# leaner-forever/SEGS-SLAM

Measured on AMD Instinct MI355X. Metric: mapper train-iters/sec (fwd+bwd raster), higher is better.
Workload: dtype f32; 1 GPU; 1080p_3m: 3000000 Gaussians, 1920x1080, 1 keyframe per GPU, fwd+bwd raster; P=3000000, P_visible=2096178, num_rendered=10472370, instances_binned=7913347, instances_live=6766534, width=1920, height=1080, parallelism=keyframe-dp1, forward=resident (no host sync), hipgraph=off

## Files before the change

### include/segs_raster.h

```cpp
#ifndef SEGS_RASTER_H_
#define SEGS_RASTER_H_

#include <stddef.h>
#include <stdint.h>

#ifdef __cplusplus
extern "C" {
#endif

#define SEGS_OK 0
#define SEGS_ERR_INVALID_ARGUMENT (-1)
#define SEGS_ERR_UNSUPPORTED (-2)
#define SEGS_ERR_ALLOC (-3)

typedef char* (*segs_alloc_fn)(void* ctx, size_t bytes);

const char* segs_last_error(void);

#define SEGS_RASTER_SKIP_NONPOSITIVE_OPACITY 1u
#define SEGS_RASTER_KEEP_DEAD_INSTANCES 2u
#define SEGS_RASTER_GATHER_TILES_TOUCHED 4u
#define SEGS_RASTER_TEST_NARROW_PACK 8u
#define SEGS_RASTER_UNFUSED_BINNING 16u
#define SEGS_RASTER_TIGHT_BINNING 32u
#define SEGS_RASTER_MFMA_MOMENTS 64u
#define SEGS_RASTER_NO_WRITTEN_BYTES 128u
uint32_t segs_raster_set_flags(uint32_t flags);

uint32_t* segs_raster_set_status_mirror(uint32_t* host_mapped_status);

size_t segs_geometry_bytes(int P);
size_t segs_image_bytes(int width, int height);
size_t segs_binning_bytes(int num_rendered);

int segs_rasterize_forward(segs_alloc_fn geometry_alloc, void* geometry_ctx,
                           segs_alloc_fn binning_alloc, void* binning_ctx,
                           segs_alloc_fn image_alloc, void* image_ctx,
                           int P, int D, int M,
                           const float* background, int width, int height,
                           const float* means3D, const float* shs, const float* colors_precomp,
                           const float* opacities, const float* scales, float scale_modifier,
                           const float* rotations, const float* cov3D_precomp,
                           const float* viewmatrix, const float* projmatrix, const float* cam_pos,
                           float tan_fovx, float tan_fovy, int prefiltered,
                           float* out_color, int* radii, void* stream, int* num_rendered);

int segs_rasterize_backward(int P, int D, int M, int R,
                            const float* background, int width, int height,
                            const float* means3D, const float* shs, const float* colors_precomp,
                            const float* scales, float scale_modifier, const float* rotations,
                            const float* cov3D_precomp, const float* viewmatrix, const float* projmatrix,
                            const float* campos, float tan_fovx, float tan_fovy, const int* radii,
                            char* geom_buffer, char* binning_buffer, char* image_buffer,
                            const float* dL_dpix, float* dL_dmean2D, float* dL_dconic, float* dL_dopacity,
                            float* dL_dcolor, float* dL_dmean3D, float* dL_dcov3D, float* dL_dsh,
                            float* dL_dscale, float* dL_drot, void* stream);

int segs_visible_filter(int P, int M, int width, int height, const float* means3D, const float* scales,
                        float scale_modifier, const float* rotations, const float* cov3D_precomp,
// ... 167 lines not shown
```

### segs-slam_amd/csrc/capi.hip

```cpp
#include <hip/hip_runtime.h>
#include <cstdio>
#include <cstdlib>
#include <algorithm>
#include <cstring>
#include <string>
#include <vector>
#include "../../include/segs_raster.h"
#include "gs_layout.h"
#include "kernels.h"
#include "capi_args.h"

using namespace segs;

namespace {
thread_local std::string g_err;
}
int segs::set_error(int code, const char* what) {
  g_err = what;
  return code;
}
int segs::set_hip_error(hipError_t e, const char* where) {
  g_err = std::string(where) + ": " + hipGetErrorString(e);
  return (int)e > 0 ? (int)e : 1;
}
// ... 261 lines not shown
      S.ranges(), S.point_list(), V.width, V.height, S.G.rec(), background, S.final_T(), S.n_contrib(), dL_dpix, S.G.gacc(), V.tiles, written);
  LAUNCH_TRY("render_bwd_kernel");
  return SEGS_OK;
}

int camera_grads_begin(const segs_camera_grads* cam, const float* shs, bool empty, hipStream_t st, bool* live) {
  *live = false;
  if (!cam) return SEGS_OK;
  if (!cam->dL_dviewmatrix || !cam->dL_dprojmatrix || !cam->temp) return fail(SEGS_ERR_INVALID_ARGUMENT, "segs_camera_grads: null field");
  if (shs) return fail(SEGS_ERR_INVALID_ARGUMENT, "camera gradients need colors_precomp: the SH colours depend on campos, which they do not cover");
  if (empty) {
    HIP_TRY(hipMemsetAsync(cam->dL_dviewmatrix, 0, 16 * sizeof(float), st));
    HIP_TRY(hipMemsetAsync(cam->dL_dprojmatrix, 0, 16 * sizeof(float), st));
    return SEGS_OK;
  }
  *live = true;
  return SEGS_OK;
}
float* camera_partials(const segs_camera_grads* cam) { return (float*)align_ptr(cam->temp); }
int camera_grads_finish(const segs_camera_grads* cam, int nblocks, hipStream_t st) {
  camera_grad_reduce_kernel<<<1, 960, 0, st>>>(camera_partials(cam), nblocks, cam->dL_dviewmatrix, cam->dL_dprojmatrix);
  LAUNCH_TRY("camera_grad_reduce_kernel");
  return SEGS_OK;
}

int launch_preprocess_bwd(const Gaussians& g, const View& V, const int* radii, const GradOutputs& o, const PerGaussianBwd& m, hipStream_t st) {
  const bool depth = m.depth || m.dz_in;
  auto* const kernel = m.cam ? (depth ? preprocess_bwd_kernel<true, true> : preprocess_bwd_kernel<false, true>)
                             : (depth ? preprocess_bwd_kernel<true, false> : preprocess_bwd_kernel<false, false>);
  const int nblocks = (g.P + 255) / 256;
  kernel<<<nblocks, 256, 0, st>>>(g.P, g.means3D, radii, g.kernel_scales(), g.rotations, g.scale_modifier, g.cov3D_precomp, V.viewmatrix,
                                  V.projmatrix, V.focal_x, V.focal_y, V.tan_fovx, V.tan_fovy, m.gacc, (float)V.width, (float)V.height,
                                  o.dL_dmean2D, o.dL_dconic, o.dL_dopacity, o.dL_dcolor, o.dL_dmean3D, o.dL_dcov3D, o.dL_dscale, o.dL_drot,
                                  m.clean_gacc ? 1 : 0, m.dz_in, m.cam ? camera_partials(m.cam) : nullptr, m.written);
  LAUNCH_TRY("preprocess_bwd_kernel");
  return m.cam ? camera_grads_finish(m.cam, nblocks, st) : SEGS_OK;
}

int rasterize_forward(const Allocators& A, const Gaussians& g, const View& V, const float* background, float* out_color, int* radii,
                      const segs_depth_outputs* dout, hipStream_t st, int* num_rendered) {
  const int P = g.P;
  if (!A.geometry_alloc || !A.binning_alloc || !A.image_alloc) return fail(SEGS_ERR_INVALID_ARGUMENT, "null allocator callback");
  if (P < 0 || V.width <= 0 || V.height <= 0) return fail(SEGS_ERR_INVALID_ARGUMENT, "bad P / image size");
  if (P > MAX_GAUSSIANS) return fail(SEGS_ERR_INVALID_ARGUMENT, "P exceeds 2^28 Gaussians (sort values carry a 4-bit quadrant mask)");
  if (!background || !out_color || !V.viewmatrix || !V.projmatrix || !num_rendered) return fail(SEGS_ERR_INVALID_ARGUMENT, "null required pointer");
  if (P > 0 && (!g.means3D || !g.opacities)) return fail(SEGS_ERR_INVALID_ARGUMENT, "null means3D/opacities");
  if (P > 0)
    if (int rc = check_colour_and_shape(g, V)) return rc;
  if (int rc = check_tile_grid(V)) return rc;

  Scratch S{};
  char* geom_raw = A.geometry_alloc(A.geometry_ctx, geom_layout(P).total);
  S.IL = image_layout(V.width, V.height);
  char* img_raw = A.image_alloc(A.image_ctx, S.IL.total);
  if (!geom_raw || !img_raw) return fail(SEGS_ERR_ALLOC, "allocator callback returned null");
  S.G = geom_at(geom_raw, P);
  S.img = align_ptr(img_raw);
  const Geom& G = S.G;
  if (!radii) radii = G.radii_internal();

  int R = 0;
  uint32_t hdr[3] = {0u, 0u, 0u};
  const bool tight = (g_flags & SEGS_RASTER_TIGHT_BINNING) != 0u;
  bool fast_keys = tight;
  if (P > 0) {
    K1Targets k1;
    k1.extra_flags = tight ? PREPROCESS_TIGHT_RECT : 0u;
// ... 62 lines not shown
  }
  if (int rc = run_binning(S, V, BinningMode::resident_keys(keys.keys, drop_dead_instances()), st)) return rc;
  return launch_render_fwd(S, V, background, out_color, dout, st);
}

int rasterize_backward(const Gaussians& g, const View& V, const ScratchBuffers& B, const BackwardInputs& in, const GradOutputs& o,
                       GaccCleaning cleaning, hipStream_t st) {
  const int P = g.P, R = B.capacity;
  const bool self_clean = cleaning == SELF_CLEAN;
  if (P < 0 || R < 0 || V.width <= 0 || V.height <= 0) return fail(SEGS_ERR_INVALID_ARGUMENT, "bad sizes");
  if (B.geom_rows < P) return fail(SEGS_ERR_INVALID_ARGUMENT, "geom_rows must be >= P");
  bool cam_live = false;
  if (int rc = camera_grads_begin(in.cam, g.shs, P == 0 || R == 0, st, &cam_live)) return rc;
  if (P == 0) return SEGS_OK;
  if (g.shs && (!V.cam_pos || !o.dL_dsh || g.M <= 0)) return fail(SEGS_ERR_INVALID_ARGUMENT, "SH path needs campos, dL_dsh and M > 0");
  if (!B.geom_buffer || !B.binning_buffer || !B.image_buffer || !in.dL_dpix || !in.background || !g.means3D || !V.viewmatrix || !V.projmatrix)
    return fail(SEGS_ERR_INVALID_ARGUMENT, "null required pointer");
  if (!o.dL_dmean2D || !o.dL_dopacity || !o.dL_dcolor || !o.dL_dmean3D || (g.cov3D_precomp && !o.dL_dcov3D))
    return fail(SEGS_ERR_INVALID_ARGUMENT, "null gradient output");
  if (!g.cov3D_precomp && (!g.scales || !g.rotations || !o.dL_dscale || !o.dL_drot))
    return fail(SEGS_ERR_INVALID_ARGUMENT, "need scales+rotations (+ their gradient outputs) or cov3D_precomp");
  uint32_t* const no_status = nullptr;
  const Scratch S = carve(B, P, V, no_status);
  const Geom& G = S.G;
  const int* radii = in.radii ? in.radii : G.radii_internal();

  if (!self_clean) { PROF(K_MEMSET);
  HIP_TRY(hipMemsetAsync(G.gacc(), 0, (size_t)P * GACC_DWORDS * 4, st));
  }
  PerGaussianBwd m;
  m.gacc = G.gacc(); m.depth = in.dgrad && in.dgrad->dL_ddepth; m.clean_gacc = self_clean;
  if (cam_live) m.cam = in.cam;
  m.written = (self_clean && !(g_flags & SEGS_RASTER_NO_WRITTEN_BYTES)) ? G.written() : nullptr;
  if (R > 0)
    if (int rc = launch_render_bwd(S, V, in.background, in.dL_dpix, in.dgrad, m.written, st)) return rc;
  { PROF(K_PREPROCESS_BWD);
  if (int rc = launch_preprocess_bwd(g, V, radii, o, m, st)) return rc;
  }
  if (g.shs) {
    sh_backward_kernel<<<G.L.nblocks, 256, 0, st>>>(P, g.means3D, radii, g.shs, g.D, g.M, V.cam_pos, G.clamped(), o.dL_dcolor, o.dL_dmean3D, o.dL_dsh);
    LAUNCH_TRY("sh_backward_kernel");
  }
  return SEGS_OK;
}

int visible_filter(const Gaussians& g, const View& V, int log_scale_stride, int* radii, hipStream_t st) {
  if (g.P < 0 || V.width <= 0 || V.height <= 0) return fail(SEGS_ERR_INVALID_ARGUMENT, "bad sizes");
  if (g.P == 0) return SEGS_OK;
  if (!g.means3D || !V.viewmatrix || !V.projmatrix || !radii) return fail(SEGS_ERR_INVALID_ARGUMENT, "null required pointer");
  if (!g.cov3D_precomp && (!g.scales || !g.rotations)) return fail(SEGS_ERR_INVALID_ARGUMENT, "need scales+rotations or cov3D_precomp");
  visible_filter_kernel<<<(g.P + 255) / 256, 256, 0, st>>>(g.P, g.means3D, g.kernel_scales(), g.scale_modifier, g.rotations, g.cov3D_precomp,
                                                           V.viewmatrix, V.projmatrix, V.width, V.height, V.tan_fovx, V.tan_fovy, V.focal_x,
                                                           V.focal_y, V.gx, V.gy, radii, log_scale_stride);
  LAUNCH_TRY("visible_filter_kernel");
  return SEGS_OK;
}

int debug_preprocess_backward(const Gaussians& g, const View& V, const int* radii, const GradOutputs& o, const float* dL_dz,
                              const segs_camera_grads* cam, hipStream_t st) {
  bool cam_live = false;
  if (int rc = camera_grads_begin(cam, g.shs, g.P <= 0, st, &cam_live)) return rc;
  if (g.P <= 0) return SEGS_OK;
  if (!g.means3D || !radii || !V.viewmatrix || !V.projmatrix || !o.dL_dmean2D || !o.dL_dconic || !o.dL_dmean3D || !o.dL_dcov3D)
    return fail(SEGS_ERR_INVALID_ARGUMENT, "null pointer");
  PerGaussianBwd m;
  if (cam_live) { m.dz_in = dL_dz; m.cam = cam; }
  return launch_preprocess_bwd(g, V, radii, o, m, st);
}

}

extern "C" {

const char* segs_last_error(void) { return g_err.c_str(); }

uint32_t* segs_raster_set_status_mirror(uint32_t* host_mapped_status) {
  uint32_t* old = g_status_mirror;
  g_status_mirror = host_mapped_status;
  return old;
}

uint32_t segs_raster_set_flags(uint32_t flags) {
  const uint32_t old = g_flags;
  g_flags = flags;
  return old;
}

size_t segs_geometry_bytes(int P) { return geom_layout(P < 0 ? 0 : P).total; }
size_t segs_image_bytes(int width, int height) { return image_layout(width, height).total; }

int segs_debug_geometry_layout(int P, size_t* offset_and_bytes, int regions) {
  if (P < 0 || !offset_and_bytes || regions != SEGS_GEOMETRY_REGIONS) return fail(SEGS_ERR_INVALID_ARGUMENT, "bad P / region count");
  const GeomLayout g = geom_layout(P);
  const size_t p = (size_t)P;
  const size_t v[SEGS_GEOMETRY_REGIONS][2] = {
      {g.rec, p * REC_DWORDS * 4}, {g.bin, p * sizeof(BinInfo)}, {g.offsets, p * 4}, {g.radii_internal, p * 4},
      {g.block_sums, (size_t)(g.nblocks + 1) * 4 * 3}, {g.clamped, p * 4}, {g.num_rendered, 64}, {g.gacc, p * GACC_DWORDS * 4},
      {g.touched, p * 4}, {g.written, p}};
  for (int i = 0; i < SEGS_GEOMETRY_REGIONS; i++) { offset_and_bytes[2 * i] = v[i][0]; offset_and_bytes[2 * i + 1] = v[i][1]; }
// ... 382 lines not shown
```

### segs-slam_amd/csrc/capi_args.h

```cpp
#pragma once
#include <hip/hip_runtime.h>
#include <cstdint>
#include "../../include/segs_raster.h"
#include "gs_layout.h"
#include "kernels.h"

namespace segs {

struct Gaussians {
  int P; const float *means3D, *scales; float scale_modifier; const float *rotations, *cov3D_precomp;
  int D, M; const float *shs, *colors_precomp, *opacities;
  const float* kernel_scales() const { return cov3D_precomp ? nullptr : scales; }
};

struct View {
  int width, height; const float *viewmatrix, *projmatrix, *cam_pos; float tan_fovx, tan_fovy;
  uint32_t gx, gy, tiles; float focal_x, focal_y;
};
inline View image_view(int width, int height) {
  View v{};
  v.width = width; v.height = height;
  v.gx = (width + TILE_X - 1) / TILE_X; v.gy = (height + TILE_Y - 1) / TILE_Y; v.tiles = v.gx * v.gy;
  return v;
}
// ... 74 lines not shown
struct BinningMode {
  uint32_t dmin; int dbits; uint32_t dcull;
  int digit_bits;
  const uint32_t* k1_keys;
  bool drop_dead;
  static constexpr int RESIDENT_DIGIT_BITS = 9;
  static BinningMode resident_keys(const uint32_t* k1_keys, bool drop_dead) {
    return BinningMode{DEPTH_KEY_MIN, DEPTH_KEY_BITS, 0xFFFFFFFFu, RESIDENT_DIGIT_BITS, k1_keys, drop_dead};
  }
  static BinningMode exact_range(uint32_t max_not_depth, uint32_t max_depth, bool drop_dead) {
    const uint32_t dmin = ~max_not_depth, dspan = max_depth - dmin + 1u;
    int dbits = 1;
    while (dbits < 32 && (dspan >> dbits) != 0u) dbits++;
    const bool nine = (dbits + 8) / 9 < (dbits + 7) / 8;
    return BinningMode{dmin, dbits, dmin + dspan, nine ? 9 : 8, nullptr, drop_dead};
  }
};
inline DepthSortInput resident_depth_sort_input(char* bin, const GaussSortLayout& GS) { return depth_sort_input(bin, GS, DEPTH_KEY_BITS, BinningMode::RESIDENT_DIGIT_BITS); }

struct K1Targets {
  uint32_t *depth_keys = nullptr, *depth_vals = nullptr;
  uint2* ranges = nullptr;
  uint32_t extra_flags = 0u;
  uint32_t* depth_overflow = nullptr;
};

struct PerGaussianBwd {
  float* gacc = nullptr;
  bool depth = false;
  bool clean_gacc = false;
  const float* dz_in = nullptr;
  const segs_camera_grads* cam = nullptr;
  uint8_t* written = nullptr;
};

struct Allocators { segs_alloc_fn geometry_alloc; void* geometry_ctx; segs_alloc_fn binning_alloc; void* binning_ctx; segs_alloc_fn image_alloc; void* image_ctx; };

enum GaccCleaning { MEMSET_PER_CALL, SELF_CLEAN };
struct BackwardInputs { const float* background; const int* radii; const float* dL_dpix; const segs_depth_grads* dgrad; const segs_camera_grads* cam; };

constexpr const Gaussians* K1_RAN_AT_PRODUCER = nullptr;
constexpr const segs_depth_outputs* NO_DEPTH_OUTPUTS = nullptr;
constexpr const segs_depth_grads* NO_DEPTH_GRADS = nullptr;
constexpr const segs_camera_grads* NO_CAMERA_GRADS = nullptr;
constexpr const float *NO_CAM_POS = nullptr, *NO_DL_DZ = nullptr;
constexpr int* NO_RADII = nullptr;

}
```

### segs-slam_amd/csrc/kernels.h

```cpp
#pragma once
#include <hip/hip_runtime.h>
#include <cstdint>
#include "gs_layout.h"

namespace segs {

int set_error(int code, const char* what);
int set_hip_error(hipError_t e, const char* where);


__global__ void preprocess_fwd_kernel(
    int P, const float* __restrict__ means3D, const float* __restrict__ scales, float mod,
    const float* __restrict__ rotations, const float* __restrict__ opacities, const float* __restrict__ colors,
    const float* __restrict__ cov3D_precomp, const float* __restrict__ viewmatrix, const float* __restrict__ projmatrix,
    int W, int H, float tan_fovx, float tan_fovy, float focal_x, float focal_y, uint32_t gx, uint32_t gy,
    int* __restrict__ radii, float* __restrict__ rec, BinInfo* __restrict__ bin, uint32_t* __restrict__ block_sums,
    uint32_t* __restrict__ depth_range, const float* __restrict__ shs, int D, int M, const float* __restrict__ cam_pos,
    uint32_t* __restrict__ clamped, uint32_t flags, uint32_t* __restrict__ depth_keys, uint32_t* __restrict__ depth_vals,
    uint2* __restrict__ ranges, int num_tiles, uint32_t* __restrict__ depth_overflow, uint32_t* __restrict__ touched_dense);
constexpr uint32_t DEPTH_KEY_MIN = 0x3E4CCCCDu;
constexpr int DEPTH_KEY_BITS = 27;

__global__ void visible_filter_kernel(
    int P, const float* __restrict__ means3D, const float* __restrict__ scales, float mod,
    const float* __restrict__ rotations, const float* __restrict__ cov3D_precomp,
    const float* __restrict__ viewmatrix, const float* __restrict__ projmatrix, int W, int H,
    float tan_fovx, float tan_fovy, float focal_x, float focal_y, uint32_t gx, uint32_t gy, int* __restrict__ radii,
    int log_scale_stride);

__global__ void mark_visible_kernel(int P, const float* __restrict__ means3D, const float* __restrict__ viewmatrix,
                                    uint8_t* __restrict__ present);

constexpr int CAM_SUMS = 24;
template <bool DEPTH, bool CAM>
__global__ void preprocess_bwd_kernel(
    int P, const float* __restrict__ means3D, const int* __restrict__ radii, const float* __restrict__ scales,
    const float* __restrict__ rotations, float mod, const float* __restrict__ cov3D_precomp,
    const float* __restrict__ view, const float* __restrict__ proj, float h_x, float h_y, float tan_fovx, float tan_fovy,
    float* __restrict__ gacc, float img_w, float img_h,
    float* __restrict__ dL_dmean2D, float* __restrict__ dL_dconic,
    float* __restrict__ dL_dopacity, float* __restrict__ dL_dcolor, float* __restrict__ dL_dmean3D,
    float* __restrict__ dL_dcov3D, float* __restrict__ dL_dscale, float* __restrict__ dL_drot, int clean_gacc,
    const float* __restrict__ dz_in, float* __restrict__ cam_partials, uint8_t* __restrict__ written);
__global__ void camera_grad_reduce_kernel(const float* __restrict__ partials, int nblocks, float* __restrict__ dL_dview,
                                          float* __restrict__ dL_dproj);
__global__ void sh_backward_kernel(int P, const float* __restrict__ means3D, const int* __restrict__ radii,
                                   const float* __restrict__ shs, int D, int M, const float* __restrict__ cam_pos,
                                   const uint32_t* __restrict__ clamped, const float* __restrict__ dL_dcolor,
                                   float* __restrict__ dL_dmean3D, float* __restrict__ dL_dsh);

__global__ void scan_block_sums_kernel(uint32_t* __restrict__ block_sums, int nblocks, const uint32_t* __restrict__ depth_range,
                                       uint32_t* __restrict__ total);
__global__ void ordered_offsets_kernel(int P, const uint32_t* __restrict__ block_sums, uint32_t* __restrict__ incl,
                                       uint32_t* __restrict__ total_out, const uint32_t* __restrict__ ng_dev,
                                       uint32_t* __restrict__ first_owner, uint32_t owner_entries);
__global__ void duplicate_with_keys_kernel(int P, int R, const float* __restrict__ rec,
                                           const uint32_t* __restrict__ order, const uint32_t* __restrict__ incl,
                                           uint32_t* __restrict__ keys, uint32_t* __restrict__ vals, uint32_t gx,
                                           const uint32_t* __restrict__ n_dev, int mark_dead, const uint32_t* __restrict__ ng_dev,
                                           const uint32_t* __restrict__ first_owner);
constexpr uint32_t RANGE_EMPTY_START = 0xFFFFFFFFu;
__global__ void normalize_ranges_kernel(int num_tiles, uint2* __restrict__ ranges);
constexpr uint32_t PREPROCESS_TIGHT_RECT = 0x80000000u;
constexpr uint32_t DEAD_KEY = 0xFFFFFFFFu;
template <typename K, int BITS>
__global__ void radix_count_kernel(const K* __restrict__ keys, int n, int shift, uint32_t dmin, int dbits,
                                   uint32_t* __restrict__ tile_prefix, uint32_t* __restrict__ chunk_hist, int nblocks, int nchunks,
                                   const uint32_t* __restrict__ n_dev, int drop_dead, int chunk_tiles, int nbits);
__global__ void radix_scan_kernel(uint32_t* __restrict__ block_hist, int nblocks, uint32_t* __restrict__ digit_totals);
template <typename K, int BITS, bool AUX>
__global__ void radix_scatter_kernel(const K* __restrict__ keys_in, const uint32_t* __restrict__ vals_in,
                                     K* __restrict__ keys_out, uint32_t* __restrict__ vals_out, int n, int shift,
                                     uint32_t dmin, int dbits, const uint32_t* __restrict__ tile_prefix, const uint32_t* __restrict__ chunk_prefix,
                                     const uint32_t* __restrict__ digit_totals, int nblocks, int nchunks,
                                     const uint32_t* __restrict__ n_dev, int drop_dead, uint32_t* __restrict__ n_live_out,
                                     const uint32_t* __restrict__ aux_in, uint32_t* __restrict__ aux_out, int nbits, int chunk_tiles, int pack_shift,
// ... 47 lines not shown
```

### segs-slam_amd/csrc/preprocess.hip

```cpp
#include <hip/hip_runtime.h>
#include <cstdint>
#include "gs_layout.h"
#include "kernels.h"
#include "project_gaussian.h"
#include "sh_color.h"

#pragma clang fp contract(off)

namespace segs {

__device__ __forceinline__ float3 load_row3(const float* __restrict__ a, int P, float* lds ) {
  const int tid = threadIdx.x;
  const size_t base = (size_t)blockIdx.x * 768;
  const size_t lim = (size_t)P * 3;
#pragma unroll
  for (int k = 0; k < 3; k++) {
    const size_t i = base + k * 256 + tid;
    lds[k * 256 + tid] = i < lim ? a[i] : 0.f;
  }
  __syncthreads();
  float3 v = make_float3(lds[3 * tid], lds[3 * tid + 1], lds[3 * tid + 2]);
  __syncthreads();
  return v;
}

__device__ __forceinline__ void load_rows3(const float* __restrict__ a0, const float* __restrict__ a1, const float* __restrict__ a2,
                                           int P, float* lds , float3& v0, float3& v1, float3& v2) {
  const int tid = threadIdx.x;
  const size_t base = (size_t)blockIdx.x * 768;
  const size_t lim = (size_t)P * 3;
  const float* arr[3] = {a0, a1, a2};
  float t[3][3];
#pragma unroll
  for (int m = 0; m < 3; m++)
#pragma unroll
    for (int k = 0; k < 3; k++) {
      const size_t i = base + k * 256 + tid;
      t[m][k] = (arr[m] && i < lim) ? arr[m][i] : 0.f;
    }
#pragma unroll
  for (int m = 0; m < 3; m++)
#pragma unroll
    for (int k = 0; k < 3; k++) lds[m * 768 + k * 256 + tid] = t[m][k];
  __syncthreads();
  v0 = make_float3(lds[3 * tid], lds[3 * tid + 1], lds[3 * tid + 2]);
  v1 = make_float3(lds[768 + 3 * tid], lds[768 + 3 * tid + 1], lds[768 + 3 * tid + 2]);
  v2 = make_float3(lds[1536 + 3 * tid], lds[1536 + 3 * tid + 1], lds[1536 + 3 * tid + 2]);
  __syncthreads();
}

__global__ void __launch_bounds__(256) preprocess_fwd_kernel(
    int P, const float* __restrict__ means3D, const float* __restrict__ scales, float mod,
    const float* __restrict__ rotations, const float* __restrict__ opacities, const float* __restrict__ colors,
    const float* __restrict__ cov3D_precomp, const float* __restrict__ viewmatrix, const float* __restrict__ projmatrix,
    int W, int H, float tan_fovx, float tan_fovy, float focal_x, float focal_y, uint32_t gx, uint32_t gy,
    int* __restrict__ radii, float* __restrict__ rec, BinInfo* __restrict__ bin, uint32_t* __restrict__ block_sums,
    uint32_t* __restrict__ depth_range ,
    const float* __restrict__ shs, int D, int M, const float* __restrict__ cam_pos, uint32_t* __restrict__ clamped,
    uint32_t flags, uint32_t* __restrict__ depth_keys, uint32_t* __restrict__ depth_vals, uint2* __restrict__ ranges,
    int num_tiles, uint32_t* __restrict__ depth_overflow ,
    uint32_t* __restrict__ touched_dense) {
  __shared__ float lds[3 * 768];
  __shared__ uint32_t wave_sums[4], wave_dmax[4], wave_dnmin[4];
  const int idx = blockIdx.x * 256 + threadIdx.x;
  float4 rot = make_float4(0, 0, 0, 0);
  if (scales && idx < P) rot = reinterpret_cast<const float4*>(rotations)[idx];
  float3 p, sc, col;
  load_rows3(means3D, scales, colors, P, lds, p, sc, col);

  uint32_t touched = 0, dbits_mine = 0;
  float4 rq0 = make_float4(0, 0, 0, 0), rq1 = rq0, rq2 = rq0, rq3 = rq0;
  bool has_record = false;
  if (idx < P) {
    Projected g = project_gaussian(p, sc, mod, rot, cov3D_precomp ? cov3D_precomp + (size_t)6 * idx : nullptr,
                                   viewmatrix, projmatrix, W, H, tan_fovx, tan_fovy, focal_x, focal_y, gx, gy);
    if ((flags & 1u) && !(opacities[idx] > 0.f)) g.radius = 0;
    BinInfo b{0u, 0u, 0u, 0u};
    if (g.radius > 0) {
      const float op = opacities[idx];
      if (!colors) {
        uint32_t cb;
        col = sh::to_rgb(idx, D, M, p, cam_pos, shs, &cb);
// ... 92 lines not shown
__global__ void __launch_bounds__(256) mark_visible_kernel(int P, const float* __restrict__ means3D,
                                                           const float* __restrict__ viewmatrix, uint8_t* __restrict__ present) {
  __shared__ float lds[768];
  const int idx = blockIdx.x * 256 + threadIdx.x;
  const float3 p = load_row3(means3D, P, lds);
  if (idx >= P) return;
  float3 p_view = transformPoint4x3(p, viewmatrix);
  present[idx] = (p_view.z <= 0.2f) ? 0 : 1;
}

__device__ __forceinline__ void store_row3(float* __restrict__ a, int P, float* lds , float x, float y, float z) {
  const int tid = threadIdx.x;
  lds[3 * tid] = x; lds[3 * tid + 1] = y; lds[3 * tid + 2] = z;
  __syncthreads();
  const size_t base = (size_t)blockIdx.x * 768;
  const size_t lim = (size_t)P * 3;
#pragma unroll
  for (int k = 0; k < 3; k++) {
    const size_t i = base + k * 256 + tid;
    if (i < lim) a[i] = lds[k * 256 + tid];
  }
  __syncthreads();
}

struct Sym2 { float xx, xy, yy; };

__device__ __forceinline__ void quat_rows(float4 q, float R[3][3]) {
  const float r = q.x, x = q.y, y = q.z, z = q.w;
  R[0][0] = 1.f - 2.f * (y * y + z * z); R[0][1] = 2.f * (x * y - r * z);       R[0][2] = 2.f * (x * z + r * y);
  R[1][0] = 2.f * (x * y + r * z);       R[1][1] = 1.f - 2.f * (x * x + z * z); R[1][2] = 2.f * (y * z - r * x);
  R[2][0] = 2.f * (x * z - r * y);       R[2][1] = 2.f * (y * z + r * x);       R[2][2] = 1.f - 2.f * (x * x + y * y);
}

template <bool DEPTH, bool CAM>
__global__ void __launch_bounds__(256) preprocess_bwd_kernel(
    int P, const float* __restrict__ means3D, const int* __restrict__ radii, const float* __restrict__ scales,
    const float* __restrict__ rotations, float mod, const float* __restrict__ cov3D_precomp,
    const float* __restrict__ view, const float* __restrict__ proj, float h_x, float h_y, float tan_fovx, float tan_fovy,
    float* __restrict__ gacc, float img_w, float img_h,
    float* __restrict__ dL_dmean2D, float* __restrict__ dL_dconic,
    float* __restrict__ dL_dopacity, float* __restrict__ dL_dcolor, float* __restrict__ dL_dmean3D,
    float* __restrict__ dL_dcov3D, float* __restrict__ dL_dscale, float* __restrict__ dL_drot,
    int clean_gacc ,
    const float* __restrict__ dz_in, float* __restrict__ cam_partials ,
    uint8_t* __restrict__ written) {
  __shared__ float lds[3 * 768];
  const int idx = blockIdx.x * 256 + threadIdx.x;
  const bool live = idx < P;
  const bool row_written = (gacc && written) ? (live && written[idx] != 0) : live;
  const bool binned = live && radii[idx] > 0 && row_written;
  float3 mean, scale, unused;
  load_rows3(means3D, scales, nullptr, P, lds, mean, scale, unused);

  float g2x = 0.f, g2y = 0.f;
  Sym2 G{0.f, 0.f, 0.f};
  float dcol0 = 0.f, dcol1 = 0.f, dcol2 = 0.f, dop = 0.f, dz = 0.f;
  float4 a0 = make_float4(0.f, 0.f, 0.f, 0.f), a1 = a0;
  if (gacc) {
    {
      __shared__ __attribute__((aligned(16))) float gl[4][32 * GACC_DWORDS];
      const int lane = threadIdx.x & 63;
      float* const wl = gl[threadIdx.x >> 6];
      const uint64_t rows = __ballot(written ? row_written : binned);
      const size_t wave_first = (size_t)blockIdx.x * 256 + (threadIdx.x & ~63);
      if (written && clean_gacc && rows != 0ull && lane < 16 && wave_first + 4 * lane < (size_t)P)
        reinterpret_cast<uint32_t*>(written + wave_first)[lane] = 0u;
#pragma unroll
      for (int half = 0; half < 2; half++) {
        float4 q[2];
#pragma unroll
        for (int j = 0; j < 2; j++) {
          const int r = 16 * j + (lane >> 2), owner = 32 * half + r;
          q[j] = make_float4(0.f, 0.f, 0.f, 0.f);
          if (((rows >> owner) & 1ull) && (lane & 3) < 3) {
            float4* src = reinterpret_cast<float4*>(gacc + (wave_first + owner) * GACC_DWORDS) + (lane & 3);
            q[j] = *src;
            if (clean_gacc) *src = make_float4(0.f, 0.f, 0.f, 0.f);
          }
        }
#pragma unroll
        for (int j = 0; j < 2; j++) reinterpret_cast<float4*>(wl + (16 * j + (lane >> 2)) * GACC_DWORDS)[lane & 3] = q[j];
        asm volatile("" ::: "memory");
        if ((lane >> 5) == half) {
          const float4* mine = reinterpret_cast<const float4*>(wl + (lane & 31) * GACC_DWORDS);
          a0 = mine[0]; a1 = mine[1]; dcol2 = wl[(lane & 31) * GACC_DWORDS + 8];
          if (DEPTH) dz = wl[(lane & 31) * GACC_DWORDS + 9];
        }
        asm volatile("" ::: "memory");
      }
    }
    if (binned) {
      G.xx = -0.5f * a0.z; G.xy = -0.5f * a0.w; G.yy = -0.5f * a1.x;
      dop = a1.y;
      dcol0 = a1.z; dcol1 = a1.w;
    }
    store_row3(dL_dcolor, P, lds, dcol0, dcol1, dcol2);
    if (live) {
      if (dL_dconic) reinterpret_cast<float4*>(dL_dconic)[idx] = make_float4(G.xx, G.xy, 0.f, G.yy);
      dL_dopacity[idx] = dop;
    }
  } else if (live) {
    g2x = dL_dmean2D[3 * (size_t)idx + 0]; g2y = dL_dmean2D[3 * (size_t)idx + 1];
    G.xx = dL_dconic[4 * (size_t)idx + 0]; G.xy = dL_dconic[4 * (size_t)idx + 1]; G.yy = dL_dconic[4 * (size_t)idx + 3];
    if constexpr (CAM && DEPTH) { if (dz_in) dz = dz_in[idx]; }
  }

  float out_mean[3] = {0, 0, 0}, out_cov[6] = {0, 0, 0, 0, 0, 0}, out_scale[3] = {0, 0, 0}, out_rot[4] = {0, 0, 0, 0};
  float cam[CAM ? CAM_SUMS : 1] = {0};
  if (binned) {
    const float tx0 = view[0] * mean.x + view[4] * mean.y + view[8] * mean.z + view[12];
    const float ty0 = view[1] * mean.x + view[5] * mean.y + view[9] * mean.z + view[13];
    const float tz = view[2] * mean.x + view[6] * mean.y + view[10] * mean.z + view[14];
    const float limx = 1.3f * tan_fovx, limy = 1.3f * tan_fovy;
    const float rx = tx0 / tz, ry = ty0 / tz;
    const bool free_x = !(rx < -limx || rx > limx), free_y = !(ry < -limy || ry > limy);
    const float tx = fminf(limx, fmaxf(-limx, rx)) * tz, ty = fminf(limy, fmaxf(-limy, ry)) * tz;
    const float iz = 1.f / tz, iz2 = iz * iz;
    const float J00 = h_x * iz, J02 = -h_x * tx * iz2, J11 = h_y * iz, J12 = -h_y * ty * iz2;
    float M2[2][3];
#pragma unroll
    for (int j = 0; j < 3; j++) {
      M2[0][j] = J00 * view[4 * j] + J02 * view[4 * j + 2];
      M2[1][j] = J11 * view[4 * j + 1] + J12 * view[4 * j + 2];
    }
    float R[3][3] = {{0, 0, 0}, {0, 0, 0}, {0, 0, 0}}, s3[3] = {0, 0, 0};
    float4 q = make_float4(0, 0, 0, 0);
    float E[2][3];
    float U[2][3] = {{0, 0, 0}, {0, 0, 0}};
    float a, b, c;
    if (cov3D_precomp) {
      const float* cv = cov3D_precomp + (size_t)6 * idx;
      const float S[3][3] = {{cv[0], cv[1], cv[2]}, {cv[1], cv[3], cv[4]}, {cv[2], cv[4], cv[5]}};
#pragma unroll
      for (int r = 0; r < 2; r++)
#pragma unroll
        for (int j = 0; j < 3; j++) E[r][j] = M2[r][0] * S[0][j] + M2[r][1] * S[1][j] + M2[r][2] * S[2][j];
      a = E[0][0] * M2[0][0] + E[0][1] * M2[0][1] + E[0][2] * M2[0][2] + 0.3f;
      b = E[0][0] * M2[1][0] + E[0][1] * M2[1][1] + E[0][2] * M2[1][2];
      c = E[1][0] * M2[1][0] + E[1][1] * M2[1][1] + E[1][2] * M2[1][2] + 0.3f;
    } else {
      q = reinterpret_cast<const float4*>(rotations)[idx];
      quat_rows(q, R);
      s3[0] = mod * scale.x; s3[1] = mod * scale.y; s3[2] = mod * scale.z;
#pragma unroll
      for (int r = 0; r < 2; r++)
#pragma unroll
        for (int k = 0; k < 3; k++) U[r][k] = (M2[r][0] * R[0][k] + M2[r][1] * R[1][k] + M2[r][2] * R[2][k]) * s3[k];
#pragma unroll
      for (int r = 0; r < 2; r++)
#pragma unroll
        for (int j = 0; j < 3; j++) E[r][j] = U[r][0] * R[j][0] * s3[0] + U[r][1] * R[j][1] * s3[1] + U[r][2] * R[j][2] * s3[2];
      a = U[0][0] * U[0][0] + U[0][1] * U[0][1] + U[0][2] * U[0][2] + 0.3f;
      b = U[0][0] * U[1][0] + U[0][1] * U[1][1] + U[0][2] * U[1][2];
      c = U[1][0] * U[1][0] + U[1][1] * U[1][1] + U[1][2] * U[1][2] + 0.3f;
    }
    const float det = a * c - b * b;
    const float k = 1.0f / (det * det + 0.0000001f);
    if (gacc) {
      const float di = 1.0f / det;
      const float cA = c * di, cB = -b * di, cC = a * di;
      g2x = -(cA * a0.x + cB * a0.y) * (0.5f * img_w);
      g2y = -(cC * a0.y + cB * a0.x) * (0.5f * img_h);
    }
    const float h0 = c * G.xx - b * G.xy, h1 = c * G.xy - b * G.yy;
    const float h2 = a * G.xy - b * G.xx, h3 = a * G.yy - b * G.xy;
    Sym2 Dc;
    Dc.xx = -k * (h0 * c - h1 * b);
    Dc.xy = -k * (h1 * a - h0 * b);
    Dc.yy = -k * (h3 * a - h2 * b);
    float DM[2][3];
#pragma unroll
    for (int j = 0; j < 3; j++) { DM[0][j] = Dc.xx * M2[0][j] + Dc.xy * M2[1][j]; DM[1][j] = Dc.xy * M2[0][j] + Dc.yy * M2[1][j]; }
    if (dL_dcov3D || cov3D_precomp) {
      const int ii[6] = {0, 0, 0, 1, 1, 2}, jj[6] = {0, 1, 2, 1, 2, 2};
// ... 41 lines not shown
        cam[3 * j + 0] = dtx * pm[j] + J00 * dM2[0][j];
        cam[3 * j + 1] = dty * pm[j] + J11 * dM2[1][j];
        cam[3 * j + 2] = dtz_all * pm[j] + (J02 * dM2[0][j] + J12 * dM2[1][j]);
        cam[12 + 3 * j + 0] = dh0 * pm[j];
        cam[12 + 3 * j + 1] = dh1 * pm[j];
        cam[12 + 3 * j + 2] = dh3 * pm[j];
      }
      cam[9] = dtx; cam[10] = dty; cam[11] = dtz_all;
      cam[21] = dh0; cam[22] = dh1; cam[23] = dh3;
    }
    if (scales) {
      float DU[2][3];
#pragma unroll
      for (int kk = 0; kk < 3; kk++) { DU[0][kk] = Dc.xx * U[0][kk] + Dc.xy * U[1][kk]; DU[1][kk] = Dc.xy * U[0][kk] + Dc.yy * U[1][kk]; }
      float GR[3][3];
#pragma unroll
      for (int kk = 0; kk < 3; kk++) {
        float ds = 0.f;
#pragma unroll
        for (int i = 0; i < 3; i++) {
          const float dLik = 2.f * (M2[0][i] * DU[0][kk] + M2[1][i] * DU[1][kk]);
          ds += R[i][kk] * dLik;
          GR[i][kk] = dLik * s3[kk];
        }
        out_scale[kk] = ds;
      }
      const float r = q.x, x = q.y, y = q.z, z = q.w;
      out_rot[0] = 2.f * (z * (GR[1][0] - GR[0][1]) + y * (GR[0][2] - GR[2][0]) + x * (GR[2][1] - GR[1][2]));
      out_rot[1] = 2.f * (y * (GR[0][1] + GR[1][0]) + z * (GR[0][2] + GR[2][0]) + r * (GR[2][1] - GR[1][2])) - 4.f * x * (GR[1][1] + GR[2][2]);
      out_rot[2] = 2.f * (x * (GR[0][1] + GR[1][0]) + r * (GR[0][2] - GR[2][0]) + z * (GR[1][2] + GR[2][1])) - 4.f * y * (GR[0][0] + GR[2][2]);
      out_rot[3] = 2.f * (r * (GR[1][0] - GR[0][1]) + x * (GR[0][2] + GR[2][0]) + y * (GR[1][2] + GR[2][1])) - 4.f * z * (GR[0][0] + GR[1][1]);
    }
  }
  if constexpr (CAM) {
    const int v = threadIdx.x >> 5, l = threadIdx.x & 31;
#pragma unroll
    for (int pass = 0; pass < CAM_SUMS / 8; pass++) {
#pragma unroll
      for (int k = 0; k < 8; k++) lds[k * 256 + threadIdx.x] = cam[pass * 8 + k];
      __syncthreads();
      float s = lds[v * 256 + l];
#pragma unroll
      for (int q = 1; q < 8; q++) s += lds[v * 256 + l + 32 * q];
#pragma unroll
      for (int off = 16; off > 0; off >>= 1) s += __shfl_down(s, off, 64);
      if (l == 0) cam_partials[(size_t)blockIdx.x * CAM_SUMS + pass * 8 + v] = s;
      __syncthreads();
    }
  }
  if (gacc) store_row3(dL_dmean2D, P, lds, g2x, g2y, 0.f);
  store_row3(dL_dmean3D, P, lds, out_mean[0], out_mean[1], out_mean[2]);
  if (dL_dscale) store_row3(dL_dscale, P, lds, out_scale[0], out_scale[1], out_scale[2]);
  if (!live) return;
  if (dL_dcov3D) {
#pragma unroll
    for (int e = 0; e < 6; e++) dL_dcov3D[6 * (size_t)idx + e] = out_cov[e];
  }
  if (dL_drot) reinterpret_cast<float4*>(dL_drot)[idx] = make_float4(out_rot[0], out_rot[1], out_rot[2], out_rot[3]);
}

#define SEGS_PREPROCESS_BWD_ARGS int, const float*, const int*, const float*, const float*, float, const float*, const float*, \
    const float*, float, float, float, float, float*, float, float, float*, float*, float*, float*, float*, float*, float*, float*, int, \
    const float*, float*, uint8_t*
template __global__ void preprocess_bwd_kernel<false, false>(SEGS_PREPROCESS_BWD_ARGS);
template __global__ void preprocess_bwd_kernel<true, false>(SEGS_PREPROCESS_BWD_ARGS);
template __global__ void preprocess_bwd_kernel<false, true>(SEGS_PREPROCESS_BWD_ARGS);
template __global__ void preprocess_bwd_kernel<true, true>(SEGS_PREPROCESS_BWD_ARGS);
#undef SEGS_PREPROCESS_BWD_ARGS

__global__ void __launch_bounds__(960) camera_grad_reduce_kernel(const float* __restrict__ partials, int nblocks,
                                                                 float* __restrict__ dL_dview, float* __restrict__ dL_dproj) {
  __shared__ float rows[160 * CAM_SUMS];
  __shared__ float mid[10 * CAM_SUMS];
  __shared__ float sums[CAM_SUMS];
  const int t = threadIdx.x, q = t % 6, r0 = t / 6;
  float4 acc = make_float4(0.f, 0.f, 0.f, 0.f);
#pragma unroll 8
  for (int r = r0; r < nblocks; r += 160) {
    const float4 x = reinterpret_cast<const float4*>(partials + (size_t)r * CAM_SUMS)[q];
    acc.x += x.x; acc.y += x.y; acc.z += x.z; acc.w += x.w;
  }
  reinterpret_cast<float4*>(rows + r0 * CAM_SUMS)[q] = acc;
  __syncthreads();
  if (t < 10 * CAM_SUMS) {
    const int v = t % CAM_SUMS, g = t / CAM_SUMS;
    float s = 0.f;
    for (int k = 0; k < 16; k++) s += rows[(16 * g + k) * CAM_SUMS + v];
    mid[g * CAM_SUMS + v] = s;
  }
  __syncthreads();
  if (t < CAM_SUMS) {
    float s = 0.f;
    for (int g = 0; g < 10; g++) s += mid[g * CAM_SUMS + t];
    sums[t] = s;
  }
  __syncthreads();
// ... 21 lines not shown
```

Measured before the change: 1014 iters/s.

## Compact sparse binned rows into dense lanes in preprocess backward

When a 256-thread block of preprocess_bwd has at most PACK_MAX_ROWS binned Gaussians, their inputs are staged through LDS into the first threads so the heavy covariance/rotation gradient math runs on a few dense wavefronts instead of scattered lanes. Results are scattered back through LDS for the existing coalesced stores. The change also hoists the rotation/cov3D loads ahead of the row-transpose wait and swizzles the gacc LDS transpose to reduce bank conflicts. It adds LDS traffic and two extra barriers per block, and is disabled on the camera-gradient path.

```diff
diff --git a/include/segs_raster.h b/include/segs_raster.h
--- a/include/segs_raster.h
+++ b/include/segs_raster.h
@@ -25,6 +25,7 @@
 #define SEGS_RASTER_TIGHT_BINNING 32u
 #define SEGS_RASTER_MFMA_MOMENTS 64u
 #define SEGS_RASTER_NO_WRITTEN_BYTES 128u
+#define SEGS_RASTER_NO_PACKED_BACKWARD 256u
 uint32_t segs_raster_set_flags(uint32_t flags);
 
 uint32_t* segs_raster_set_status_mirror(uint32_t* host_mapped_status);
diff --git a/segs-slam_amd/csrc/capi.hip b/segs-slam_amd/csrc/capi.hip
--- a/segs-slam_amd/csrc/capi.hip
+++ b/segs-slam_amd/csrc/capi.hip
@@ -317,7 +317,7 @@
   kernel<<<nblocks, 256, 0, st>>>(g.P, g.means3D, radii, g.kernel_scales(), g.rotations, g.scale_modifier, g.cov3D_precomp, V.viewmatrix,
                                   V.projmatrix, V.focal_x, V.focal_y, V.tan_fovx, V.tan_fovy, m.gacc, (float)V.width, (float)V.height,
                                   o.dL_dmean2D, o.dL_dconic, o.dL_dopacity, o.dL_dcolor, o.dL_dmean3D, o.dL_dcov3D, o.dL_dscale, o.dL_drot,
-                                  m.clean_gacc ? 1 : 0, m.dz_in, m.cam ? camera_partials(m.cam) : nullptr, m.written);
+                                  m.clean_gacc ? 1 : 0, m.dz_in, m.cam ? camera_partials(m.cam) : nullptr, m.written, m.cam ? 0 : m.pack_max);
   LAUNCH_TRY("preprocess_bwd_kernel");
   return m.cam ? camera_grads_finish(m.cam, nblocks, st) : SEGS_OK;
 }
@@ -446,6 +446,7 @@
   m.gacc = G.gacc(); m.depth = in.dgrad && in.dgrad->dL_ddepth; m.clean_gacc = self_clean;
   if (cam_live) m.cam = in.cam;
   m.written = (self_clean && !(g_flags & SEGS_RASTER_NO_WRITTEN_BYTES)) ? G.written() : nullptr;
+  m.pack_max = (g_flags & SEGS_RASTER_NO_PACKED_BACKWARD) ? 0 : PACK_MAX_ROWS;
   if (R > 0)
     if (int rc = launch_render_bwd(S, V, in.background, in.dL_dpix, in.dgrad, m.written, st)) return rc;
   { PROF(K_PREPROCESS_BWD);
@@ -479,6 +480,7 @@
     return fail(SEGS_ERR_INVALID_ARGUMENT, "null pointer");
   PerGaussianBwd m;
   if (cam_live) { m.dz_in = dL_dz; m.cam = cam; }
+  m.pack_max = (g_flags & SEGS_RASTER_NO_PACKED_BACKWARD) ? 0 : PACK_MAX_ROWS;
   return launch_preprocess_bwd(g, V, radii, o, m, st);
 }
 
diff --git a/segs-slam_amd/csrc/capi_args.h b/segs-slam_amd/csrc/capi_args.h
--- a/segs-slam_amd/csrc/capi_args.h
+++ b/segs-slam_amd/csrc/capi_args.h
@@ -130,6 +130,7 @@
   const float* dz_in = nullptr;
   const segs_camera_grads* cam = nullptr;
   uint8_t* written = nullptr;
+  int pack_max = 0;
 };
 
 struct Allocators { segs_alloc_fn geometry_alloc; void* geometry_ctx; segs_alloc_fn binning_alloc; void* binning_ctx; segs_alloc_fn image_alloc; void* image_ctx; };
diff --git a/segs-slam_amd/csrc/kernels.h b/segs-slam_amd/csrc/kernels.h
--- a/segs-slam_amd/csrc/kernels.h
+++ b/segs-slam_amd/csrc/kernels.h
@@ -41,7 +41,11 @@
     float* __restrict__ dL_dmean2D, float* __restrict__ dL_dconic,
     float* __restrict__ dL_dopacity, float* __restrict__ dL_dcolor, float* __restrict__ dL_dmean3D,
     float* __restrict__ dL_dcov3D, float* __restrict__ dL_dscale, float* __restrict__ dL_drot, int clean_gacc,
-    const float* __restrict__ dz_in, float* __restrict__ cam_partials, uint8_t* __restrict__ written);
+    const float* __restrict__ dz_in, float* __restrict__ cam_partials, uint8_t* __restrict__ written, int pack_max);
+#ifndef SEGS_PACK_MAX_ROWS
+#define SEGS_PACK_MAX_ROWS 64
+#endif
+constexpr int PACK_MAX_ROWS = SEGS_PACK_MAX_ROWS;
 __global__ void camera_grad_reduce_kernel(const float* __restrict__ partials, int nblocks, float* __restrict__ dL_dview,
                                           float* __restrict__ dL_dproj);
 __global__ void sh_backward_kernel(int P, const float* __restrict__ means3D, const int* __restrict__ radii,
diff --git a/segs-slam_amd/csrc/preprocess.hip b/segs-slam_amd/csrc/preprocess.hip
--- a/segs-slam_amd/csrc/preprocess.hip
+++ b/segs-slam_amd/csrc/preprocess.hip
@@ -24,13 +24,12 @@
   return v;
 }
 
-__device__ __forceinline__ void load_rows3(const float* __restrict__ a0, const float* __restrict__ a1, const float* __restrict__ a2,
-                                           int P, float* lds , float3& v0, float3& v1, float3& v2) {
+__device__ __forceinline__ void issue_rows3(const float* __restrict__ a0, const float* __restrict__ a1, const float* __restrict__ a2,
+                                            int P, float (&t)[3][3]) {
   const int tid = threadIdx.x;
   const size_t base = (size_t)blockIdx.x * 768;
   const size_t lim = (size_t)P * 3;
   const float* arr[3] = {a0, a1, a2};
-  float t[3][3];
 #pragma unroll
   for (int m = 0; m < 3; m++)
 #pragma unroll
@@ -38,6 +37,9 @@
       const size_t i = base + k * 256 + tid;
       t[m][k] = (arr[m] && i < lim) ? arr[m][i] : 0.f;
     }
+}
+__device__ __forceinline__ void finish_rows3(const float (&t)[3][3], float* lds , float3& v0, float3& v1, float3& v2) {
+  const int tid = threadIdx.x;
 #pragma unroll
   for (int m = 0; m < 3; m++)
 #pragma unroll
@@ -48,6 +50,14 @@
   v2 = make_float3(lds[1536 + 3 * tid], lds[1536 + 3 * tid + 1], lds[1536 + 3 * tid + 2]);
   __syncthreads();
 }
+__device__ __forceinline__ void load_rows3(const float* __restrict__ a0, const float* __restrict__ a1, const float* __restrict__ a2,
+                                           int P, float* lds , float3& v0, float3& v1, float3& v2) {
+  float t[3][3];
+  issue_rows3(a0, a1, a2, P, t);
+  finish_rows3(t, lds, v0, v1, v2);
+}
+
+__device__ __forceinline__ int row_swizzle_load(int r) { return (r >> 2) & 3; }
 
 __global__ void __launch_bounds__(256) preprocess_fwd_kernel(
     int P, const float* __restrict__ means3D, const float* __restrict__ scales, float mod,
@@ -206,6 +216,9 @@
   R[2][0] = 2.f * (x * z - r * y);       R[2][1] = 2.f * (y * z + r * x);       R[2][2] = 1.f - 2.f * (x * x + y * y);
 }
 
+constexpr int PACK_OUT0 = 3, PACK_OUT_FIELDS = 18;
+constexpr int BWD_LDS_FLOATS = (PACK_OUT0 + PACK_OUT_FIELDS) * 256;
+static_assert(BWD_LDS_FLOATS >= 3 * 768 + 4 * 32 * GACC_DWORDS, "the sweeps' staging and the four waves' row transposes sit side by side");
 template <bool DEPTH, bool CAM>
 __global__ void __launch_bounds__(256) preprocess_bwd_kernel(
     int P, const float* __restrict__ means3D, const int* __restrict__ radii, const float* __restrict__ scales,
@@ -217,14 +230,46 @@
     float* __restrict__ dL_dcov3D, float* __restrict__ dL_dscale, float* __restrict__ dL_drot,
     int clean_gacc ,
     const float* __restrict__ dz_in, float* __restrict__ cam_partials ,
-    uint8_t* __restrict__ written) {
-  __shared__ float lds[3 * 768];
+    uint8_t* __restrict__ written, int pack_max) {
+  __shared__ __attribute__((aligned(16))) float shm[BWD_LDS_FLOATS];
+  __shared__ uint32_t wave_rows[4];
+  float* const lds = shm;
   const int idx = blockIdx.x * 256 + threadIdx.x;
+  const int lane = threadIdx.x & 63, wave = __builtin_amdgcn_readfirstlane(threadIdx.x >> 6);
   const bool live = idx < P;
-  const bool row_written = (gacc && written) ? (live && written[idx] != 0) : live;
-  const bool binned = live && radii[idx] > 0 && row_written;
+  const bool by_byte = gacc && written;
+  const int row = live ? idx : P - 1;
+  int mark = by_byte ? (int)written[row] : radii[row];
+  float sweeps[3][3];
+  issue_rows3(means3D, scales, nullptr, P, sweeps);
+  asm volatile("" : "+v"(mark));
+  const bool binned = live && mark > 0;
+  const uint64_t bmask = __ballot(binned);
+  if (lane == 0) wave_rows[wave] = (uint32_t)__popcll(bmask);
+  float4 q;
+  {
+    typedef float float4_any __attribute__((ext_vector_type(4), aligned(4)));
+    const int first = bmask ? (int)(blockIdx.x * 256 + (threadIdx.x & ~63)) + __builtin_ctzll(bmask) : 0;
+    const size_t qrow = binned ? idx : first;
+    const float* const src = cov3D_precomp ? cov3D_precomp + 6 * qrow : rotations + 4 * qrow;
+    const float4_any v = *reinterpret_cast<const float4_any*>(src);
+    q = make_float4(v.x, v.y, v.z, v.w);
+  }
   float3 mean, scale, unused;
-  load_rows3(means3D, scales, nullptr, P, lds, mean, scale, unused);
+  finish_rows3(sweeps, lds, mean, scale, unused);
+  if (binned && cov3D_precomp) {
+    const float* cv = cov3D_precomp + (size_t)6 * idx;
+    scale = make_float3(cv[4], cv[5], 0.f);
+  }
+  uint32_t slot = __builtin_amdgcn_mbcnt_hi((uint32_t)(bmask >> 32), __builtin_amdgcn_mbcnt_lo((uint32_t)bmask, 0u)), total = 0;
+#pragma unroll
+  for (int w = 0; w < 4; w++) {
+    const uint32_t c = wave_rows[w];
+    slot += w < wave ? c : 0u;
+    total += c;
+  }
+  total = __builtin_amdgcn_readfirstlane(total);
+  const bool packed = !CAM && total != 0u && total <= (uint32_t)pack_max;
 
   float g2x = 0.f, g2y = 0.f;
   Sym2 G{0.f, 0.f, 0.f};
@@ -232,33 +277,38 @@
   float4 a0 = make_float4(0.f, 0.f, 0.f, 0.f), a1 = a0;
   if (gacc) {
     {
-      __shared__ __attribute__((aligned(16))) float gl[4][32 * GACC_DWORDS];
-      const int lane = threadIdx.x & 63;
-      float* const wl = gl[threadIdx.x >> 6];
-      const uint64_t rows = __ballot(written ? row_written : binned);
+      float* const wl = shm + 3 * 768 + wave * (32 * GACC_DWORDS);
+      const uint64_t rows = bmask;
       const size_t wave_first = (size_t)blockIdx.x * 256 + (threadIdx.x & ~63);
       if (written && clean_gacc && rows != 0ull && lane < 16 && wave_first + 4 * lane < (size_t)P)
         reinterpret_cast<uint32_t*>(written + wave_first)[lane] = 0u;
 #pragma unroll
       for (int half = 0; half < 2; half++) {
-        float4 q[2];
+        float4 qr[2];
 #pragma unroll
         for (int j = 0; j < 2; j++) {
           const int r = 16 * j + (lane >> 2), owner = 32 * half + r;
-          q[j] = make_float4(0.f, 0.f, 0.f, 0.f);
+          qr[j] = make_float4(0.f, 0.f, 0.f, 0.f);
           if (((rows >> owner) & 1ull) && (lane & 3) < 3) {
             float4* src = reinterpret_cast<float4*>(gacc + (wave_first + owner) * GACC_DWORDS) + (lane & 3);
-            q[j] = *src;
+            qr[j] = *src;
             if (clean_gacc) *src = make_float4(0.f, 0.f, 0.f, 0.f);
           }
         }
 #pragma unroll
-        for (int j = 0; j < 2; j++) reinterpret_cast<float4*>(wl + (16 * j + (lane >> 2)) * GACC_DWORDS)[lane & 3] = q[j];
+        for (int j = 0; j < 2; j++) {
+          const int r = 16 * j + (lane >> 2);
+          reinterpret_cast<float4*>(wl + r * GACC_DWORDS)[(lane & 3) ^ row_swizzle_load(r)] = qr[j];
+        }
         asm volatile("" ::: "memory");
         if ((lane >> 5) == half) {
           const float4* mine = reinterpret_cast<const float4*>(wl + (lane & 31) * GACC_DWORDS);
-          a0 = mine[0]; a1 = mine[1]; dcol2 = wl[(lane & 31) * GACC_DWORDS + 8];
-          if (DEPTH) dz = wl[(lane & 31) * GACC_DWORDS + 9];
+          const int x = row_swizzle_load(lane & 31);
+          a0 = mine[0 ^ x]; a1 = mine[1 ^ x];
+          float4 a2 = mine[2 ^ x];
+          asm volatile("" : "+v"(a2.x), "+v"(a2.y), "+v"(a2.z), "+v"(a2.w));
+          dcol2 = a2.x;
+          if (DEPTH) dz = a2.y;
         }
         asm volatile("" ::: "memory");
       }
@@ -281,7 +331,33 @@
 
   float out_mean[3] = {0, 0, 0}, out_cov[6] = {0, 0, 0, 0, 0, 0}, out_scale[3] = {0, 0, 0}, out_rot[4] = {0, 0, 0, 0};
   float cam[CAM ? CAM_SUMS : 1] = {0};
-  if (binned) {
+  bool work = binned;
+  if constexpr (!CAM) {
+    if (packed) {
+      if (binned) {
+        float* const s = shm + slot;
+        s[0 * 256] = mean.x; s[1 * 256] = mean.y; s[2 * 256] = mean.z;
+        s[3 * 256] = scale.x; s[4 * 256] = scale.y; s[5 * 256] = scale.z;
+        s[6 * 256] = q.x; s[7 * 256] = q.y; s[8 * 256] = q.z; s[9 * 256] = q.w;
+        s[10 * 256] = gacc ? a0.x : g2x; s[11 * 256] = gacc ? a0.y : g2y;
+        s[12 * 256] = G.xx; s[13 * 256] = G.xy; s[14 * 256] = G.yy;
+        if (DEPTH) s[15 * 256] = dz;
+      }
+      __syncthreads();
+      work = threadIdx.x < total;
+      if (work) {
+        const float* const s = shm + threadIdx.x;
+        mean = make_float3(s[0 * 256], s[1 * 256], s[2 * 256]);
+        scale = make_float3(s[3 * 256], s[4 * 256], s[5 * 256]);
+        q = make_float4(s[6 * 256], s[7 * 256], s[8 * 256], s[9 * 256]);
+        const float m0 = s[10 * 256], m1 = s[11 * 256];
+        if (gacc) { a0.x = m0; a0.y = m1; } else { g2x = m0; g2y = m1; }
+        G.xx = s[12 * 256]; G.xy = s[13 * 256]; G.yy = s[14 * 256];
+        if (DEPTH) dz = s[15 * 256];
+      }
+    }
+  }
+  if (work) {
     const float tx0 = view[0] * mean.x + view[4] * mean.y + view[8] * mean.z + view[12];
     const float ty0 = view[1] * mean.x + view[5] * mean.y + view[9] * mean.z + view[13];
     const float tz = view[2] * mean.x + view[6] * mean.y + view[10] * mean.z + view[14];
@@ -298,12 +374,11 @@
       M2[1][j] = J11 * view[4 * j + 1] + J12 * view[4 * j + 2];
     }
     float R[3][3] = {{0, 0, 0}, {0, 0, 0}, {0, 0, 0}}, s3[3] = {0, 0, 0};
-    float4 q = make_float4(0, 0, 0, 0);
     float E[2][3];
     float U[2][3] = {{0, 0, 0}, {0, 0, 0}};
     float a, b, c;
     if (cov3D_precomp) {
-      const float* cv = cov3D_precomp + (size_t)6 * idx;
+      const float cv[6] = {q.x, q.y, q.z, q.w, scale.x, scale.y};
       const float S[3][3] = {{cv[0], cv[1], cv[2]}, {cv[1], cv[3], cv[4]}, {cv[2], cv[4], cv[5]}};
 #pragma unroll
       for (int r = 0; r < 2; r++)
@@ -313,7 +388,6 @@
       b = E[0][0] * M2[1][0] + E[0][1] * M2[1][1] + E[0][2] * M2[1][2];
       c = E[1][0] * M2[1][0] + E[1][1] * M2[1][1] + E[1][2] * M2[1][2] + 0.3f;
     } else {
-      q = reinterpret_cast<const float4*>(rotations)[idx];
       quat_rows(q, R);
       s3[0] = mod * scale.x; s3[1] = mod * scale.y; s3[2] = mod * scale.z;
 #pragma unroll
@@ -421,6 +495,40 @@
       out_rot[3] = 2.f * (r * (GR[1][0] - GR[0][1]) + x * (GR[0][2] + GR[2][0]) + y * (GR[1][2] + GR[2][1])) - 4.f * z * (GR[0][0] + GR[1][1]);
     }
   }
+  if constexpr (!CAM) {
+    if (packed) {
+      if (work) {
+        float* const s = shm + PACK_OUT0 * 256 + threadIdx.x;
+        s[0 * 256] = out_mean[0]; s[1 * 256] = out_mean[1]; s[2 * 256] = out_mean[2];
+        s[3 * 256] = g2x; s[4 * 256] = g2y;
+        s[5 * 256] = out_scale[0]; s[6 * 256] = out_scale[1]; s[7 * 256] = out_scale[2];
+        s[8 * 256] = out_rot[0]; s[9 * 256] = out_rot[1]; s[10 * 256] = out_rot[2]; s[11 * 256] = out_rot[3];
+        if (dL_dcov3D) {
+#pragma unroll
+          for (int e = 0; e < 6; e++) s[(12 + e) * 256] = out_cov[e];
+        }
+      }
+      __syncthreads();
+      g2x = g2y = 0.f;
+#pragma unroll
+      for (int e = 0; e < 3; e++) out_mean[e] = out_scale[e] = 0.f;
+#pragma unroll
+      for (int e = 0; e < 4; e++) out_rot[e] = 0.f;
+#pragma unroll
+      for (int e = 0; e < 6; e++) out_cov[e] = 0.f;
+      if (binned) {
+        const float* const s = shm + PACK_OUT0 * 256 + slot;
+        out_mean[0] = s[0 * 256]; out_mean[1] = s[1 * 256]; out_mean[2] = s[2 * 256];
+        g2x = s[3 * 256]; g2y = s[4 * 256];
+        out_scale[0] = s[5 * 256]; out_scale[1] = s[6 * 256]; out_scale[2] = s[7 * 256];
+        out_rot[0] = s[8 * 256]; out_rot[1] = s[9 * 256]; out_rot[2] = s[10 * 256]; out_rot[3] = s[11 * 256];
+        if (dL_dcov3D) {
+#pragma unroll
+          for (int e = 0; e < 6; e++) out_cov[e] = s[(12 + e) * 256];
+        }
+      }
+    }
+  }
   if constexpr (CAM) {
     const int v = threadIdx.x >> 5, l = threadIdx.x & 31;
 #pragma unroll
@@ -450,7 +558,7 @@
 
 #define SEGS_PREPROCESS_BWD_ARGS int, const float*, const int*, const float*, const float*, float, const float*, const float*, \
     const float*, float, float, float, float, float*, float, float, float*, float*, float*, float*, float*, float*, float*, float*, int, \
-    const float*, float*, uint8_t*
+    const float*, float*, uint8_t*, int
 template __global__ void preprocess_bwd_kernel<false, false>(SEGS_PREPROCESS_BWD_ARGS);
 template __global__ void preprocess_bwd_kernel<true, false>(SEGS_PREPROCESS_BWD_ARGS);
 template __global__ void preprocess_bwd_kernel<false, true>(SEGS_PREPROCESS_BWD_ARGS);
```

Measured after the change: 1006 iters/s. Within noise of the previous version (-0.8%).
